# HiKapok/X-Detector

Hardware: AMD Instinct MI355X
Metric: images/sec at 480x480 Light-Head R-CNN, 1/2/4/8 MI355X + backbone MFMA util% (higher is better)
Workload: dtype f16x3 (split-precision f16 MFMA, f32 accumulate, f32 activations); 1 GPU; Full Light-Head R-CNN (Xception backbone + RPN + GPU proposals/NMS + PSROIAlign + light head + per-class NMS), 300 proposals, 480x480; batch_per_gpu=256, global_batch=256, image_size=480, concurrent_sub_batches=2, cross_terms=f16, input=whitened f32 [B,3,480,480] resident in HBM, parallelism=image-sharded dp1, weights=seeded random init (no checkpoint exists), graph_replay=True

## Files before the change

### x-detector_amd/csrc/conv_mfma_dma.hip

```cpp
#include "common.h"
#include "conv_epilogue.h"
#include <cstdlib>
#include <cstring>
#include <type_traits>

namespace xdet {

typedef float f32x16 __attribute__((ext_vector_type(16)));
typedef _Float16 f16x8 __attribute__((ext_vector_type(8)));
typedef int x8frag __attribute__((ext_vector_type(8)));
typedef int x8half __attribute__((ext_vector_type(4)));
typedef unsigned short u16;

#define XDET_GLDS16(gptr, lptr)                                                                        \
  __builtin_amdgcn_global_load_lds((const __attribute__((address_space(1))) void*)(gptr),              \
                                   (__attribute__((address_space(3))) void*)(lptr), 16, 0, 0)

template <int BM, int BN, int WAVES_M, int WAVES_N, int NSPLIT, int NSTAGE, bool PW = false, bool FOLD = false, bool X8 = false,
          bool GBUF = false>
__global__ __launch_bounds__(64 * WAVES_M * WAVES_N) void conv_dma_f16_kernel(ConvParams p_in) {
  static_assert(NSTAGE == 2, "two LDS stages");
  static_assert(!(GBUF && PW), "GBUF is the buffer form of the NON-pointwise layers");
  static_assert(!X8 || (PW && NSPLIT == 3 && !FOLD), "x8: pointwise f16x3 layers only");
  constexpr int NW = WAVES_M * WAVES_N;
  constexpr int WM = BM / WAVES_M, WN = BN / WAVES_N;
  constexpr int TM = WM / 32, TN = WN / 32;
  constexpr int A_IT = BM / (16 * NW);
  constexpr int B_IT = BN / (16 * NW);
  static_assert(A_IT >= 1 && B_IT >= 1, "tile too small for the wave count");
  constexpr int ROWB = 32;
  constexpr int STAGE = (2 * BM + 2 * BN) * ROWB;

  extern __shared__ __attribute__((aligned(16))) u16 smem16[];

  const int tid = threadIdx.x;
  const int lane = tid & 63;
  const int wave = __builtin_amdgcn_readfirstlane(tid >> 6);
  const int wm = wave / WAVES_N, wn = wave % WAVES_N;
  const int nby = p_in.Cout_pad / BN;
  const int slot = blockIdx.x >> 3;
  int bx, n0;
  ConvParams p = p_in;
  if (p_in.group_rows) {
    const int mt = p_in.group_rows / BM;
    const int tpg = mt * nby;
    const int g = (slot / tpg) * 8 + (blockIdx.x & 7);
    const int w = slot - (slot / tpg) * tpg;
    if ((int64_t)g * p_in.group_rows >= p_in.M) return;
    if (p_in.group_live_rows && (w / nby) * BM >= p_in.group_live_rows) return;
    bx = g * mt + w / nby;
    n0 = (w % nby) * BN;
    p.wt_hi = p_in.wt_hi + (size_t)g * p_in.group_wt_stride;
    p.wt_lo = p_in.wt_lo ? p_in.wt_lo + (size_t)g * p_in.group_wt_stride : nullptr;
    p.scale = p_in.scale + (size_t)g * p_in.Cout_pad;
    p.shift = p_in.shift + (size_t)g * p_in.Cout_pad;
  } else {
    bx = (slot / nby) * 8 + (blockIdx.x & 7);
    if (bx * BM >= p_in.M) return;
    n0 = (slot % nby) * BN;
  }
  const int m0 = bx * BM;

  const int lr = lane >> 2;
  const int pos = lane & 3;
  int iy0[A_IT], ix0[A_IT], pbase[A_IT], achunk[A_IT];
#pragma unroll
  for (int q = 0; q < A_IT; ++q) {
    const int rt = (wave * A_IT + q) * 16 + lr;
    achunk[q] = (pos ^ ((rt >> 2) & 3)) * 8;
    const int m = m0 + rt;
    if (m < p.M) {
      const int hw = p.Ho * p.Wo;
      const int n = m / hw;
      const int rem = m - n * hw;
      const int oy = rem / p.Wo;
      const int ox = rem - oy * p.Wo;
      iy0[q] = oy * p.stride - p.pad_t;
      ix0[q] = ox * p.stride - p.pad_l;
      pbase[q] = n * p.H * p.W;
    } else {
      iy0[q] = -(1 << 20);
      ix0[q] = 0;
      pbase[q] = 0;
    }
  }
  size_t boff[B_IT];
#pragma unroll
  for (int q = 0; q < B_IT; ++q) {
    const int rt = (wave * B_IT + q) * 16 + lr;
    boff[q] = (size_t)(n0 + rt) * 32 + (pos ^ ((rt >> 2) & 3)) * 8;
  }
  const int nk = p.Kp / 32;
  const int ntaps = p.KH * p.KW;
  const unsigned c32n = (unsigned)(p.ldi >> 5);

  __amdgpu_buffer_rsrc_t r_ah, r_al, r_bh, r_bl;
  unsigned a_vo[A_IT], b_vo[B_IT];
  int g_cc = 0, g_ky = 0, g_kx = 0, g_tap = 0;
  if (GBUF) {
    const unsigned a_bytes = (unsigned)(((size_t)(((size_t)p.N * p.H * p.W + 15) >> 4) * c32n) << 10);
    const unsigned b_bytes = (unsigned)((size_t)nk * p.Cout_pad * 64);
    r_ah = __builtin_amdgcn_make_buffer_rsrc(const_cast<u16*>(p.in_hi), 0, (int)a_bytes, 0x00020000);
    r_al = __builtin_amdgcn_make_buffer_rsrc(const_cast<u16*>(NSPLIT > 1 ? p.in_lo : p.in_hi), 0, (int)a_bytes, 0x00020000);
    r_bh = __builtin_amdgcn_make_buffer_rsrc(const_cast<u16*>(p.wt_hi), 0, (int)b_bytes, 0x00020000);
    r_bl = __builtin_amdgcn_make_buffer_rsrc(const_cast<u16*>(NSPLIT > 1 ? p.wt_lo : p.wt_hi), 0, (int)b_bytes, 0x00020000);
#pragma unroll
    for (int q = 0; q < B_IT; ++q) b_vo[q] = (unsigned)(boff[q] * 2);
  }
  if (PW) {
    const unsigned a_bytes = (unsigned)(((size_t)((p.M + 15) >> 4) * c32n) << 10);
    const unsigned b_bytes = (unsigned)((size_t)nk * p.Cout_pad * 64);
    r_ah = __builtin_amdgcn_make_buffer_rsrc(const_cast<u16*>(p.in_hi), 0, (int)a_bytes, 0x00020000);
    r_al = __builtin_amdgcn_make_buffer_rsrc(const_cast<u16*>(NSPLIT > 1 ? p.in_lo : p.in_hi), 0, (int)a_bytes, 0x00020000);
    r_bh = __builtin_amdgcn_make_buffer_rsrc(const_cast<u16*>(p.wt_hi), 0, (int)b_bytes, 0x00020000);
    r_bl = __builtin_amdgcn_make_buffer_rsrc(const_cast<u16*>(NSPLIT > 1 ? p.wt_lo : p.wt_hi), 0, (int)b_bytes, 0x00020000);
#pragma unroll
    for (int q = 0; q < A_IT; ++q) {
      const int rt = (wave * A_IT + q) * 16 + lr;
      const int m = m0 + rt;
      a_vo[q] = m < p.M ? (((unsigned)(m >> 4) * c32n) << 10) + (unsigned)((((m & 15) << 5) + achunk[q]) * 2) : 0xffffffffu;
    }
#pragma unroll
    for (int q = 0; q < B_IT; ++q) b_vo[q] = (unsigned)(boff[q] * 2);
  }

  auto issue = [&](int kt, int buf) {
    u16* Ah = smem16 + buf * STAGE;
    u16* Al = Ah + BM * ROWB;
    u16* Bh = Al + BM * ROWB;
    u16* Bl = Bh + BN * ROWB;
    if (PW) {
      const unsigned a_so = (unsigned)kt << 10;
      const unsigned b_so = (unsigned)kt * (unsigned)p.Cout_pad * 64u;
#pragma unroll
      for (int q = 0; q < A_IT; ++q) {
        __builtin_amdgcn_raw_ptr_buffer_load_lds(r_ah, (__attribute__((address_space(3))) void*)(Ah + (wave * A_IT + q) * 16 * ROWB),
                                                 16, (int)a_vo[q], (int)a_so, 0, 0);
        if (NSPLIT > 1)
          __builtin_amdgcn_raw_ptr_buffer_load_lds(r_al, (__attribute__((address_space(3))) void*)(Al + (wave * A_IT + q) * 16 * ROWB),
                                                   16, (int)a_vo[q], (int)a_so, 0, 0);
      }
#pragma unroll
      for (int q = 0; q < B_IT; ++q) {
        __builtin_amdgcn_raw_ptr_buffer_load_lds(r_bh, (__attribute__((address_space(3))) void*)(Bh + (wave * B_IT + q) * 16 * ROWB),
                                                 16, (int)b_vo[q], (int)b_so, 0, 0);
        if (NSPLIT > 1)
          __builtin_amdgcn_raw_ptr_buffer_load_lds(r_bl, (__attribute__((address_space(3))) void*)(Bl + (wave * B_IT + q) * 16 * ROWB),
                                                   16, (int)b_vo[q], (int)b_so, 0, 0);
      }
    } else if (GBUF) {
      const int dy = g_ky * p.dil, dx = g_kx * p.dil;
      const unsigned a_so = (unsigned)g_cc << 10;
      const unsigned b_so = (unsigned)(g_tap * (p.Cin_p >> 5) + g_cc) * (unsigned)p.Cout_pad * 64u;
#pragma unroll
      for (int q = 0; q < A_IT; ++q) {
        const int iy = iy0[q] + dy, ix = ix0[q] + dx;
        const bool ok = (unsigned)iy < (unsigned)p.H && (unsigned)ix < (unsigned)p.W;
        const unsigned pix = (unsigned)(pbase[q] + iy * p.W + ix);
        const unsigned vo = ok ? (((pix >> 4) * c32n) << 10) + (((pix & 15) << 5) + (unsigned)achunk[q]) * 2u : 0xffffffffu;
        __builtin_amdgcn_raw_ptr_buffer_load_lds(r_ah, (__attribute__((address_space(3))) void*)(Ah + (wave * A_IT + q) * 16 * ROWB),
                                                 16, (int)vo, (int)a_so, 0, 0);
        if (NSPLIT > 1)
          __builtin_amdgcn_raw_ptr_buffer_load_lds(r_al, (__attribute__((address_space(3))) void*)(Al + (wave * A_IT + q) * 16 * ROWB),
                                                   16, (int)vo, (int)a_so, 0, 0);
      }
#pragma unroll
      for (int q = 0; q < B_IT; ++q) {
        __builtin_amdgcn_raw_ptr_buffer_load_lds(r_bh, (__attribute__((address_space(3))) void*)(Bh + (wave * B_IT + q) * 16 * ROWB),
                                                 16, (int)b_vo[q], (int)b_so, 0, 0);
        if (NSPLIT > 1)
          __builtin_amdgcn_raw_ptr_buffer_load_lds(r_bl, (__attribute__((address_space(3))) void*)(Bl + (wave * B_IT + q) * 16 * ROWB),
                                                   16, (int)b_vo[q], (int)b_so, 0, 0);
      }
      ++g_tap;
      if (++g_kx == p.KW) {
        g_kx = 0;
        if (++g_ky == p.KH) { g_ky = 0; g_tap = 0; ++g_cc; }
      }
    } else {
    const int cc = kt / ntaps;
    const int tap = kt - cc * ntaps;
    const int ky = tap / p.KW;
    const int dy = ky * p.dil, dx = (tap - ky * p.KW) * p.dil;
    const size_t k0 = (size_t)(tap * (p.Cin_p >> 5) + cc) * p.Cout_pad * 32;
#pragma unroll
    for (int q = 0; q < A_IT; ++q) {
      const int iy = iy0[q] + dy, ix = ix0[q] + dx;
      const bool ok = (unsigned)iy < (unsigned)p.H && (unsigned)ix < (unsigned)p.W;
      const unsigned pix = (unsigned)(pbase[q] + iy * p.W + ix);
      const size_t off = ((size_t)((pix >> 4) * c32n + cc) << 9) + ((pix & 15) << 5) + achunk[q];
      const u16* sh = ok ? p.in_hi + off : p.zeros;
      XDET_GLDS16(sh, Ah + (wave * A_IT + q) * 16 * ROWB);
      if (NSPLIT > 1) {
        const u16* sl = ok ? p.in_lo + off : p.zeros;
        XDET_GLDS16(sl, Al + (wave * A_IT + q) * 16 * ROWB);
      }
    }
#pragma unroll
    for (int q = 0; q < B_IT; ++q) {
      XDET_GLDS16(p.wt_hi + boff[q] + k0, Bh + (wave * B_IT + q) * 16 * ROWB);
      if (NSPLIT > 1) XDET_GLDS16(p.wt_lo + boff[q] + k0, Bl + (wave * B_IT + q) * 16 * ROWB);
    }
    }
  };

  f32x16 acc[TM][TN];
#pragma unroll
  for (int i = 0; i < TM; ++i)
#pragma unroll
    for (int j = 0; j < TN; ++j)
#pragma unroll
      for (int r = 0; r < 16; ++r) acc[i][j][r] = 0.f;

  const int frow = lane & 31;
  const int fh = lane >> 5;
  int aoff[TM], boffs[TN], asw[TM], bsw[TN];
#pragma unroll
  for (int i = 0; i < TM; ++i) {
    const int rt = wm * WM + i * 32 + frow;
    aoff[i] = rt * ROWB;
    asw[i] = (rt >> 2) & 3;
  }
#pragma unroll
  for (int j = 0; j < TN; ++j) {
    const int rt = wn * WN + j * 32 + frow;
    boffs[j] = rt * ROWB;
    bsw[j] = (rt >> 2) & 3;
  }

  f32x16 tot[FOLD ? TM : 1][FOLD ? TN : 1];
  int fold_steps = 1 << 30, next_fold = 1 << 30;
  bool first_range = true;
  if constexpr (FOLD) {
    const int ncc = p.Cin_p >> 5, S = p.ksplit > 0 ? p.ksplit : 1;
    fold_steps = ((ncc + S - 1) / S) * ntaps;
    next_fold = fold_steps;
#pragma unroll
    for (int i = 0; i < TM; ++i)
#pragma unroll
      for (int j = 0; j < TN; ++j)
#pragma unroll
        for (int r = 0; r < 16; ++r) tot[i][j][r] = 0.f;
  }
  auto main_loop = [&](auto JN_) {
  constexpr int JN = decltype(JN_)::value;
  auto load_frags = [&](int buf, int ks, f16x8* ah, f16x8* al, f16x8* bh, f16x8* bl) {
    const u16* Ah = smem16 + buf * STAGE;
    const u16* Al = Ah + BM * ROWB;
    const u16* Bh = Al + BM * ROWB;
    const u16* Bl = Bh + BN * ROWB;
    const int c = ks * 2 + fh;
#pragma unroll
    for (int i = 0; i < TM; ++i) {
      const int o = aoff[i] + ((c ^ asw[i]) << 3);
      ah[i] = *reinterpret_cast<const f16x8*>(Ah + o);
      if constexpr (NSPLIT > 1 && !X8) al[i] = *reinterpret_cast<const f16x8*>(Al + o);
    }
#pragma unroll
    for (int j = 0; j < JN; ++j) {
      const int o = boffs[j] + ((c ^ bsw[j]) << 3);
      bh[j] = *reinterpret_cast<const f16x8*>(Bh + o);
      if constexpr (NSPLIT > 1 && !X8) bl[j] = *reinterpret_cast<const f16x8*>(Bl + o);
    }
  };
  auto load_x8 = [&](int buf, x8frag* a8, x8frag* b8) {
    const u16* Al = smem16 + buf * STAGE + BM * ROWB;
    const u16* Bl = Al + BM * ROWB + BN * ROWB;
#pragma unroll
    for (int i = 0; i < TM; ++i) {
      const x8half q0 = *reinterpret_cast<const x8half*>(Al + aoff[i] + (((2 * fh) ^ asw[i]) << 3));
      const x8half q1 = *reinterpret_cast<const x8half*>(Al + aoff[i] + (((2 * fh + 1) ^ asw[i]) << 3));
      a8[i] = x8frag{q0[0], q0[1], q0[2], q0[3], q1[0], q1[1], q1[2], q1[3]};
    }
#pragma unroll
    for (int j = 0; j < JN; ++j) {
      const x8half q0 = *reinterpret_cast<const x8half*>(Bl + boffs[j] + (((2 * fh) ^ bsw[j]) << 3));
      const x8half q1 = *reinterpret_cast<const x8half*>(Bl + boffs[j] + (((2 * fh + 1) ^ bsw[j]) << 3));
      b8[j] = x8frag{q0[0], q0[1], q0[2], q0[3], q1[0], q1[1], q1[2], q1[3]};
    }
  };
  const int x8_sa = X8 ? 127 + p.x8_exp - (fh ? 11 : 0) : 0;
  const int x8_sb = fh ? 127 + 2 : 127 - 9;
  auto mma_x8 = [&](const x8frag* a8, const x8frag* b8) {
#pragma unroll
    for (int i = 0; i < TM; ++i)
#pragma unroll
      for (int j = 0; j < JN; ++j)
        acc[i][j] = __builtin_amdgcn_mfma_scale_f32_32x32x64_f8f6f4(a8[i], b8[j], acc[i][j], 0, 0, 0, x8_sa, 0, x8_sb);
  };
  auto mma = [&](const f16x8* ah, const f16x8* al, const f16x8* bh, const f16x8* bl) {
    if constexpr (NSPLIT > 1 && !X8) {
#pragma unroll
      for (int i = 0; i < TM; ++i)
#pragma unroll
        for (int j = 0; j < JN; ++j)
          acc[i][j] = __builtin_amdgcn_mfma_f32_32x32x16_f16(al[i], bh[j], acc[i][j], 0, 0, 0);
#pragma unroll
      for (int i = 0; i < TM; ++i)
#pragma unroll
        for (int j = 0; j < JN; ++j)
          acc[i][j] = __builtin_amdgcn_mfma_f32_32x32x16_f16(ah[i], bl[j], acc[i][j], 0, 0, 0);
    }
#pragma unroll
    for (int i = 0; i < TM; ++i)
#pragma unroll
      for (int j = 0; j < JN; ++j)
        acc[i][j] = __builtin_amdgcn_mfma_f32_32x32x16_f16(ah[i], bh[j], acc[i][j], 0, 0, 0);
  };

  f16x8 a0h[TM], a0l[X8 ? 1 : TM], b0h[TN], b0l[X8 ? 1 : TN];
  f16x8 a1h[TM], a1l[X8 ? 1 : TM], b1h[TN], b1l[X8 ? 1 : TN];
  x8frag a8[X8 ? TM : 1], b8[X8 ? TN : 1];
  issue(0, 0);
  asm volatile("s_waitcnt vmcnt(0)" ::: "memory");
  __syncthreads();
  if (nk > 1) issue(1, 1);
  load_frags(0, 0, a0h, a0l, b0h, b0l);
  auto step = [&](int kt, auto steady) {
    constexpr bool STEADY = decltype(steady)::value;
    const int buf = kt & 1;
    if constexpr (FOLD) {
      if (kt == next_fold) {
#pragma unroll
        for (int i = 0; i < TM; ++i)
#pragma unroll
          for (int j = 0; j < TN; ++j) {
            tot[i][j] = first_range ? acc[i][j] : tot[i][j] + acc[i][j];
#pragma unroll
            for (int r = 0; r < 16; ++r) acc[i][j][r] = 0.f;
          }
        first_range = false;
        next_fold += fold_steps;
      }
    }
    load_frags(buf, 1, a1h, a1l, b1h, b1l);
    if constexpr (X8) load_x8(buf, a8, b8);
    __builtin_amdgcn_sched_barrier(0);
    mma(a0h, a0l, b0h, b0l);
    __builtin_amdgcn_sched_barrier(0);
    asm volatile("s_waitcnt vmcnt(0)" ::: "memory");
    __syncthreads();
    if (STEADY || kt + 1 < nk) load_frags(buf ^ 1, 0, a0h, a0l, b0h, b0l);
    if (STEADY || kt + 2 < nk) issue(kt + 2, buf);
    if (!STEADY) __builtin_amdgcn_sched_barrier(0);
    mma(a1h, a1l, b1h, b1l);
    if constexpr (X8) mma_x8(a8, b8);
    if (STEADY) {
      constexpr int NPIECE = (A_IT + B_IT) * (NSPLIT > 1 ? 2 : 1);
      constexpr int NMMA = TM * JN * (X8 ? 2 : NSPLIT > 1 ? 3 : 1);
      constexpr int NRD = (TM + JN) * (NSPLIT > 1 && !X8 ? 2 : 1);
      __builtin_amdgcn_sched_group_barrier(0x100, NRD, 0);
#pragma unroll
      for (int k = 0; k < NPIECE; ++k) {
        __builtin_amdgcn_sched_group_barrier(0x008, NMMA / NPIECE > 0 ? NMMA / NPIECE : 1, 0);
        __builtin_amdgcn_sched_group_barrier(0x010, 1, 0);
      }
    }
    __builtin_amdgcn_sched_barrier(0);
  };
  int kt = 0;
  for (; kt + 2 < nk; ++kt) step(kt, std::true_type{});
  for (; kt < nk; ++kt) step(kt, std::false_type{});
  };
  const int jn_live = (p.ldo - (n0 + wn * WN) + 31) >> 5;
  static_assert(TN == 2, "the tiles of this kernel are two column blocks per wave");
  if constexpr (PW) {
    if (jn_live == 1 && p.skip_dead != 0) main_loop(std::integral_constant<int, 1>{});
    else main_loop(std::integral_constant<int, TN>{});
  } else {
    main_loop(std::integral_constant<int, TN>{});
  }

  if constexpr (FOLD) {
    if (!first_range) {
#pragma unroll
      for (int i = 0; i < TM; ++i)
#pragma unroll
        for (int j = 0; j < TN; ++j) acc[i][j] = tot[i][j] + acc[i][j];
    }
  }
  if (m0 + BM <= p.M) conv_epilogue_full<WM, WN, TM, TN, NW, NSTAGE * STAGE * 2>(p, acc, smem16, wave, lane, wm, wn, m0, n0);
  else conv_epilogue<WM, WN, TM, TN, NW, NSTAGE * STAGE * 2>(p, acc, smem16, wave, lane, wm, wn, m0, n0);
}

template <int OFF>
__device__ __forceinline__ f16x8 cd_ds_read_b128(unsigned addr) {
  f16x8 r;
  asm volatile("ds_read_b128 %0, %1 offset:%2" : "=v"(r) : "v"(addr), "n"(OFF) : "memory");
  return r;
}

template <int NSPLIT, bool PW = false, bool W8 = false, bool H64 = false>
__global__ __launch_bounds__(W8 ? 512 : 256) void conv_dma_deep_kernel(ConvParams p_in) {
  constexpr int BM = H64 ? 64 : 128, BN = 64, NW = W8 ? 8 : 4;
  static_assert(!W8 || NSPLIT == 3, "eight waves: the f16x3 form");
  static_assert(!(W8 && H64), "64 x 64 tiles: four waves");
  constexpr bool WT = W8 || H64;
  constexpr int PAIR = 2;
  constexpr int NSTAGE = 3 * PAIR;
  constexpr int TN = WT ? 1 : 2;
  constexpr int A_IT = BM / (16 * NW), B_IT = W8 ? 1 : BN / (16 * NW);
  constexpr int ROWB = 32;
  constexpr int STAGE = (2 * BM + 2 * BN) * ROWB;
  constexpr int PIECES = W8 ? 3 : (A_IT + B_IT) * (NSPLIT > 1 ? 2 : 1);
  extern __shared__ __attribute__((aligned(16))) u16 smem16[];

  const int tid = threadIdx.x;
  const int lane = tid & 63;
  const int wave = __builtin_amdgcn_readfirstlane(tid >> 6);
  const int nby = p_in.Cout_pad / BN;
  const int slot = blockIdx.x >> 3;
  int bx, n0;
  ConvParams p = p_in;
  if (p_in.group_rows) {
    const int mt = p_in.group_rows / BM;
    const int tpg = mt * nby;
    const int g = (slot / tpg) * 8 + (blockIdx.x & 7);
    const int w = slot - (slot / tpg) * tpg;
    if ((int64_t)g * p_in.group_rows >= p_in.M) return;
    if (p_in.group_live_rows && (w / nby) * BM >= p_in.group_live_rows) return;
    bx = g * mt + w / nby;
    n0 = (w % nby) * BN;
    p.wt_hi = p_in.wt_hi + (size_t)g * p_in.group_wt_stride;
    p.wt_lo = p_in.wt_lo ? p_in.wt_lo + (size_t)g * p_in.group_wt_stride : nullptr;
    p.scale = p_in.scale + (size_t)g * p_in.Cout_pad;
    p.shift = p_in.shift + (size_t)g * p_in.Cout_pad;
  } else {
    bx = (slot / nby) * 8 + (blockIdx.x & 7);
    if (bx * BM >= p_in.M) return;
    n0 = (slot % nby) * BN;
  }
  const int m0 = bx * BM;

  const int lr = lane >> 2, pos = lane & 3;
  int iy0[A_IT], ix0[A_IT], pbase[A_IT], achunk[A_IT];
#pragma unroll
  for (int q = 0; q < A_IT; ++q) {
    const int rt = (wave * A_IT + q) * 16 + lr;
    achunk[q] = (pos ^ ((rt >> 2) & 3)) * 8;
    const int m = m0 + rt;
    if (m < p.M) {
      const int hw = p.Ho * p.Wo;
      const int n = m / hw;
      const int rem = m - n * hw;
      const int oy = rem / p.Wo;
      const int ox = rem - oy * p.Wo;
      iy0[q] = oy * p.stride - p.pad_t;
      ix0[q] = ox * p.stride - p.pad_l;
      pbase[q] = n * p.H * p.W;
    } else {
      iy0[q] = -(1 << 20);
      ix0[q] = 0;
      pbase[q] = 0;
    }
  }
  size_t boff[B_IT];
#pragma unroll
  for (int q = 0; q < B_IT; ++q) {
    const int rt = (W8 ? (wave >> 1) : wave * B_IT + q) * 16 + lr;
    boff[q] = (size_t)(n0 + rt) * 32 + (pos ^ ((rt >> 2) & 3)) * 8;
  }
  const int nk = p.Kp / 32;
  const int ntaps = p.KH * p.KW;
  const unsigned c32n = (unsigned)(p.ldi >> 5);

  unsigned a_vo[A_IT], b_vo[B_IT];
  unsigned a_bytes = 0, b_bytes = 0;
  if (PW) {
    a_bytes = (unsigned)(((size_t)((p.M + 15) >> 4) * c32n) << 10);
    b_bytes = (unsigned)((size_t)nk * p.Cout_pad * 64);
#pragma unroll
    for (int q = 0; q < A_IT; ++q) {
      const int rt = (wave * A_IT + q) * 16 + lr;
      const int m = m0 + rt;
      a_vo[q] = m < p.M ? (((unsigned)(m >> 4) * c32n) << 10) + (unsigned)((((m & 15) << 5) + achunk[q]) * 2) : 0xffffffffu;
    }
#pragma unroll
    for (int q = 0; q < B_IT; ++q) b_vo[q] = (unsigned)(boff[q] * 2);
  }

  auto issue = [&](int kt, int buf) {
    u16* Ah = smem16 + buf * STAGE;
    u16* Al = Ah + BM * ROWB;
    u16* Bh = Al + BM * ROWB;
    u16* Bl = Bh + BN * ROWB;
    const bool live = kt < nk;
    if (PW) {
      const __amdgpu_buffer_rsrc_t r_ah = __builtin_amdgcn_make_buffer_rsrc(const_cast<u16*>(p.in_hi), 0, live ? (int)a_bytes : 0, 0x00020000);
      const __amdgpu_buffer_rsrc_t r_al = __builtin_amdgcn_make_buffer_rsrc(const_cast<u16*>(NSPLIT > 1 ? p.in_lo : p.in_hi), 0, live ? (int)a_bytes : 0, 0x00020000);
      const __amdgpu_buffer_rsrc_t r_bh = __builtin_amdgcn_make_buffer_rsrc(const_cast<u16*>(p.wt_hi), 0, live ? (int)b_bytes : 0, 0x00020000);
      const __amdgpu_buffer_rsrc_t r_bl = __builtin_amdgcn_make_buffer_rsrc(const_cast<u16*>(NSPLIT > 1 ? p.wt_lo : p.wt_hi), 0, live ? (int)b_bytes : 0, 0x00020000);
      const unsigned a_so = (unsigned)kt << 10, b_so = (unsigned)kt * (unsigned)p.Cout_pad * 64u;
#pragma unroll
      for (int q = 0; q < A_IT; ++q) {
        __builtin_amdgcn_raw_ptr_buffer_load_lds(r_ah, (__attribute__((address_space(3))) void*)(Ah + (wave * A_IT + q) * 16 * ROWB), 16, (int)a_vo[q], (int)a_so, 0, 0);
        if (NSPLIT > 1)
          __builtin_amdgcn_raw_ptr_buffer_load_lds(r_al, (__attribute__((address_space(3))) void*)(Al + (wave * A_IT + q) * 16 * ROWB), 16, (int)a_vo[q], (int)a_so, 0, 0);
      }
      if constexpr (W8) {
        __builtin_amdgcn_raw_ptr_buffer_load_lds((wave & 1) ? r_bl : r_bh, (__attribute__((address_space(3))) void*)(((wave & 1) ? Bl : Bh) + (wave >> 1) * 16 * ROWB), 16,
                                                 (int)b_vo[0], (int)b_so, 0, 0);
      } else {
#pragma unroll
      for (int q = 0; q < B_IT; ++q) {
        __builtin_amdgcn_raw_ptr_buffer_load_lds(r_bh, (__attribute__((address_space(3))) void*)(Bh + (wave * B_IT + q) * 16 * ROWB), 16, (int)b_vo[q], (int)b_so, 0, 0);
        if (NSPLIT > 1)
          __builtin_amdgcn_raw_ptr_buffer_load_lds(r_bl, (__attribute__((address_space(3))) void*)(Bl + (wave * B_IT + q) * 16 * ROWB), 16, (int)b_vo[q], (int)b_so, 0, 0);
      }
      }
    } else {
    const int cc = kt / ntaps;
    const int tap = kt - cc * ntaps;
    const int ky = tap / p.KW;
    const int dy = ky * p.dil, dx = (tap - ky * p.KW) * p.dil;
    const size_t k0 = (size_t)(tap * (p.Cin_p >> 5) + cc) * p.Cout_pad * 32;
#pragma unroll
    for (int q = 0; q < A_IT; ++q) {
      const int iy = iy0[q] + dy, ix = ix0[q] + dx;
      const bool ok = live && (unsigned)iy < (unsigned)p.H && (unsigned)ix < (unsigned)p.W;
      const unsigned pix = (unsigned)(pbase[q] + iy * p.W + ix);
      const size_t off = ((size_t)((pix >> 4) * c32n + cc) << 9) + ((pix & 15) << 5) + achunk[q];
      XDET_GLDS16(ok ? p.in_hi + off : p.zeros, Ah + (wave * A_IT + q) * 16 * ROWB);
      if (NSPLIT > 1) XDET_GLDS16(ok ? p.in_lo + off : p.zeros, Al + (wave * A_IT + q) * 16 * ROWB);
    }
    if constexpr (W8) {
      XDET_GLDS16(live ? ((wave & 1) ? p.wt_lo : p.wt_hi) + boff[0] + k0 : p.zeros, ((wave & 1) ? Bl : Bh) + (wave >> 1) * 16 * ROWB);
    } else {
#pragma unroll
    for (int q = 0; q < B_IT; ++q) {
      XDET_GLDS16(live ? p.wt_hi + boff[q] + k0 : p.zeros, Bh + (wave * B_IT + q) * 16 * ROWB);
      if (NSPLIT > 1) XDET_GLDS16(live ? p.wt_lo + boff[q] + k0 : p.zeros, Bl + (wave * B_IT + q) * 16 * ROWB);
    }
    }
    }
  };

  f32x16 acc[1][TN];
#pragma unroll
  for (int j = 0; j < TN; ++j)
#pragma unroll
    for (int r = 0; r < 16; ++r) acc[0][j][r] = 0.f;

  const int frow = lane & 31, fh = lane >> 5;
  const unsigned lds0 = (unsigned)(size_t)(__attribute__((address_space(3))) void*)(smem16);
  unsigned a_off[2], b_off[2][TN];
#pragma unroll
  for (int ks = 0; ks < 2; ++ks) {
    const int c = ks * 2 + fh;
    const int ra = (WT ? (wave >> 1) : wave) * 32 + frow;
    a_off[ks] = (unsigned)(ra * ROWB + ((c ^ ((ra >> 2) & 3)) << 3)) * 2u;
#pragma unroll
    for (int j = 0; j < TN; ++j) {
      const int rb = (WT ? (wave & 1) : j) * 32 + frow;
      b_off[ks][j] = (unsigned)(2 * BM * ROWB + rb * ROWB + ((c ^ ((rb >> 2) & 3)) << 3)) * 2u;
    }
  }

#pragma unroll
  for (int q = 0; q < 2 * PAIR; ++q) issue(q, q);
  int ring = 0;
  for (int kt = 0; kt < nk; kt += PAIR) {
    asm volatile("s_waitcnt vmcnt(%0)\n\ts_barrier" ::"n"(PAIR * PIECES) : "memory");
    {
      const int ns = ring + 2 * PAIR >= NSTAGE ? ring + 2 * PAIR - NSTAGE : ring + 2 * PAIR;
#pragma unroll
      for (int q = 0; q < PAIR; ++q) issue(kt + 2 * PAIR + q, ns + q);
    }
    __builtin_amdgcn_sched_barrier(0);
#pragma unroll
    for (int q = 0; q < PAIR; ++q) {
      const unsigned sb = lds0 + (unsigned)((ring + q) * STAGE * 2);
      f16x8 ah[2], al[2], bh[2][TN], bl[2][TN];
#pragma unroll
      for (int ks = 0; ks < 2; ++ks) {
        ah[ks] = cd_ds_read_b128<0>(sb + a_off[ks]);
        if (NSPLIT > 1) al[ks] = cd_ds_read_b128<BM * ROWB * 2>(sb + a_off[ks]);
#pragma unroll
        for (int j = 0; j < TN; ++j) {
          bh[ks][j] = cd_ds_read_b128<0>(sb + b_off[ks][j]);
          if (NSPLIT > 1) bl[ks][j] = cd_ds_read_b128<BN * ROWB * 2>(sb + b_off[ks][j]);
        }
      }
#pragma unroll
      for (int ks = 0; ks < 2; ++ks) {
        if (NSPLIT > 1) asm volatile("s_waitcnt lgkmcnt(0)" : "+v"(ah[ks]), "+v"(al[ks])::"memory");
        else asm volatile("s_waitcnt lgkmcnt(0)" : "+v"(ah[ks])::"memory");
#pragma unroll
        for (int j = 0; j < TN; ++j) {
          asm volatile("" : "+v"(bh[ks][j]));
          if (NSPLIT > 1) asm volatile("" : "+v"(bl[ks][j]));
        }
      }
#pragma unroll
      for (int ks = 0; ks < 2; ++ks) {
        if (NSPLIT > 1) {
#pragma unroll
          for (int j = 0; j < TN; ++j) acc[0][j] = __builtin_amdgcn_mfma_f32_32x32x16_f16(al[ks], bh[ks][j], acc[0][j], 0, 0, 0);
#pragma unroll
          for (int j = 0; j < TN; ++j) acc[0][j] = __builtin_amdgcn_mfma_f32_32x32x16_f16(ah[ks], bl[ks][j], acc[0][j], 0, 0, 0);
        }
#pragma unroll
        for (int j = 0; j < TN; ++j) acc[0][j] = __builtin_amdgcn_mfma_f32_32x32x16_f16(ah[ks], bh[ks][j], acc[0][j], 0, 0, 0);
      }
    }
    ring = ring + PAIR >= NSTAGE ? ring + PAIR - NSTAGE : ring + PAIR;
  }
  asm volatile("s_waitcnt vmcnt(0)" ::: "memory");
  if (m0 + BM <= p.M) conv_epilogue_full<32, 32 * TN, 1, TN, NW, NSTAGE * STAGE * 2>(p, acc, smem16, wave, lane, WT ? (wave >> 1) : wave, WT ? (wave & 1) : 0, m0, n0);
  else conv_epilogue<32, 32 * TN, 1, TN, NW, NSTAGE * STAGE * 2>(p, acc, smem16, wave, lane, WT ? (wave >> 1) : wave, WT ? (wave & 1) : 0, m0, n0);
}

static bool pw_eligible(const ConvParams& p) {
  if (p.KH != 1 || p.KW != 1 || p.stride != 1 || p.pad_t != 0 || p.pad_l != 0 || p.H != p.Ho || p.W != p.Wo) return false;
  const size_t a_bytes = ((size_t)((p.M + 15) >> 4) * (size_t)(p.ldi >> 5)) << 10;
  const size_t b_bytes = (size_t)(p.Kp / 32) * p.Cout_pad * 64;
  return a_bytes < ((size_t)1 << 32) && b_bytes < ((size_t)1 << 32) && p.Cin_p == p.Kp;
}

template <int NSPLIT, bool PW = false, bool W8 = false, bool H64 = false>
static int launch_deep(const ConvParams& p, hipStream_t s) {
  if (!PW && pw_eligible(p)) return launch_deep<NSPLIT, true, W8, H64>(p, s);
  if constexpr (!W8 && !H64 && NSPLIT == 3) {
    if (!p.group_rows && cdiv(p.M, 128) * (p.Cout_pad / 64) <= 128) return launch_deep<NSPLIT, PW, false, true>(p, s);
    return launch_deep<NSPLIT, PW, true>(p, s);
  }
  constexpr int BM = H64 ? 64 : 128;
  constexpr size_t lds = (size_t)6 * (2 * BM + 2 * 64) * 32 * sizeof(u16);
  auto kern = conv_dma_deep_kernel<NSPLIT, PW, W8, H64>;
  static DeviceOnce once;
  XDET_TRY(ensure_dynamic_lds(once, reinterpret_cast<const void*>(kern), (int)lds));
  dim3 grid((unsigned)(cdiv(cdiv(p.M, BM), 8) * 8 * (p.Cout_pad / 64)));
  if (p.group_rows) {
    const int64_t groups = p.M / p.group_rows, tpg = (int64_t)(p.group_rows / BM) * (p.Cout_pad / 64);
    grid = dim3((unsigned)(cdiv(groups, 8) * 8 * tpg));
  }
  hipLaunchKernelGGL(kern, grid, dim3(W8 ? 512 : 256), lds, s, p);
  XDET_LAUNCH_CHECK();
  return XDET_OK;
}

static bool gbuf_eligible(const ConvParams& p) {
  if (p.group_rows != 0) return false;
  const size_t a_bytes = ((((size_t)p.N * p.H * p.W + 15) >> 4) * (size_t)(p.ldi >> 5)) << 10;
  const size_t b_bytes = (size_t)(p.Kp / 32) * p.Cout_pad * 64;
  return a_bytes < ((size_t)1 << 32) && b_bytes < ((size_t)1 << 32) && p.Kp == p.Cin_p * p.KH * p.KW;
}

template <int BM, int BN, int WAVES_M, int WAVES_N, int NSPLIT, int NSTAGE = 2, bool PW = false, bool X8 = false, bool GBUF = false>
static int launch_d(const ConvParams& p, hipStream_t s) {
  if (!PW && pw_eligible(p)) return launch_d<BM, BN, WAVES_M, WAVES_N, NSPLIT, NSTAGE, true>(p, s);
  if constexpr (PW && !X8 && NSPLIT == 3) {
    if (p.x8) return launch_d<BM, BN, WAVES_M, WAVES_N, NSPLIT, NSTAGE, true, true>(p, s);
  }
  XDET_REQUIRE(X8 || !p.x8, "conv(dma): x8 planes need a pointwise f16x3 layer below 4 GiB");
  constexpr size_t lds = (size_t)NSTAGE * (2 * BM + 2 * BN) * 32 * sizeof(u16);
  if constexpr (!PW && !X8 && !GBUF && BM == 256 && BN == 256) {
    if (gbuf_eligible(p)) return launch_d<BM, BN, WAVES_M, WAVES_N, NSPLIT, NSTAGE, false, false, true>(p, s);
  }
  auto kern = conv_dma_f16_kernel<BM, BN, WAVES_M, WAVES_N, NSPLIT, NSTAGE, PW, false, X8, GBUF>;
  static DeviceOnce once;
  XDET_TRY(ensure_dynamic_lds(once, reinterpret_cast<const void*>(kern), (int)lds));
  dim3 grid((unsigned)(cdiv(cdiv(p.M, BM), 8) * 8 * (p.Cout_pad / BN)));
  if (p.group_rows) {
    const int64_t groups = p.M / p.group_rows, tpg = (int64_t)(p.group_rows / BM) * (p.Cout_pad / BN);
    grid = dim3((unsigned)(cdiv(groups, 8) * 8 * tpg));
  }
  hipLaunchKernelGGL(kern, grid, dim3(64 * WAVES_M * WAVES_N), lds, s, p);
  XDET_LAUNCH_CHECK();
  return XDET_OK;
}

bool conv_dma_fold_applicable(const ConvParams& p, int n_tile, int nsplit) {
  return n_tile == 128 && nsplit == 3 && p.group_rows == 0 && p.ksplit > 1 && cdiv(p.M, 256) * (p.Cout_pad / 128) >= 170;
}
int launch_conv_mfma_dma_fold(const ConvParams& p, hipStream_t s) {
  constexpr size_t lds = (size_t)2 * (2 * 256 + 2 * 128) * 32 * sizeof(u16);
  auto kern = conv_dma_f16_kernel<256, 128, 4, 2, 3, 2, false, true>;
  static DeviceOnce once;
  XDET_TRY(ensure_dynamic_lds(once, reinterpret_cast<const void*>(kern), (int)lds));
  dim3 grid((unsigned)(cdiv(cdiv(p.M, 256), 8) * 8 * (p.Cout_pad / 128)));
  hipLaunchKernelGGL(kern, grid, dim3(512), lds, s, p);
  XDET_LAUNCH_CHECK();
  return XDET_OK;
}

int launch_conv_mfma_dma(const ConvParams& p_in, int n_tile, int nsplit, hipStream_t s) {
  ConvParams p = p_in;
  p.skip_dead = 1;
  XDET_REQUIRE(p.Kp % 32 == 0 && p.Cin_p % 32 == 0 && p.ldi >= p.Cin_p && p.ldi % 8 == 0,
               "conv(dma): channel counts must be padded to 32");
  XDET_REQUIRE(p.Cout_pad % n_tile == 0, "conv(dma): Cout_pad must be a multiple of the N tile");
  XDET_REQUIRE(p.in_hi && (nsplit == 1 || p.in_lo) && p.wt_hi && (nsplit == 1 || p.wt_lo) && p.zeros,
               "conv(dma): split planes missing");
  if (p.M <= 0) return XDET_OK;
  if (n_tile == 128 && nsplit == 3) {
    const int64_t b256 = cdiv(p.M, 256) * (p.Cout_pad / 256);
    const int nk = p.Kp / 32;
    int tile = 0;
    const bool full_rounds = b256 >= 240 && (b256 % 256 == 0 || b256 % 256 >= 240);
    if (p.Cout_pad % 256 == 0 && (b256 >= 512 || full_rounds || (b256 >= 200 && nk >= 40))) tile = 2;
    if (p.group_rows && p.group_rows % 256 != 0) tile = 0;
    if (tile == 2) return launch_d<256, 256, 2, 4, 3>(p, s);
  }
  if (n_tile == 128 && nsplit == 3 && !p.group_rows && !p.x8) {
    const int64_t b128 = cdiv(p.M, 128) * (p.Cout_pad / 128);
    if (b128 > 128 && b128 <= 256 && p.Kp / 32 >= 16 && p.Kp == p.Cin_p * p.KH * p.KW && p.ldi % 32 == 0 &&
        conv_ksplit_supported(p.KH, p.KW, (int64_t)p.N * p.H * p.W, p.ldi, p.Cin_p, p.Cout_pad)) {
      ConvParams q = p;
      q.ksplit = 1;
      q.ks_partial = nullptr;
      return launch_conv_mfma_ksplit(q, 128, 3, 2, 0, s);
    }
  }
  if (n_tile == 128 && nsplit == 3 && p.group_rows && p.group_rows % 64 == 0 && !p.x8) {
    const int live = p.group_live_rows ? p.group_live_rows : p.group_rows;
    const int64_t groups = p.M / p.group_rows, wgs = groups * cdiv(live, 64) * (p.Cout_pad / 64);
    if (live <= 64 && wgs <= 768) return launch_deep<3, false, false, true>(p, s);
  }
  if (n_tile == 128) {
    const int64_t b128 = cdiv(p.M, 128) * (p.Cout_pad / 128);
    if (nsplit == 3 && b128 <= 128 && (!p.group_rows || p.group_rows % 128 == 0)) {
      return p.x8 ? launch_d<128, 64, 4, 1, 3>(p, s) : launch_deep<3>(p, s);
    }
    return nsplit == 1 ? launch_d<128, 128, 2, 2, 1>(p, s) : launch_d<128, 128, 2, 2, 3>(p, s);
  }
  if (n_tile == 64) return nsplit == 1 ? launch_d<128, 64, 4, 1, 1>(p, s) : launch_d<128, 64, 4, 1, 3>(p, s);
  set_last_error("conv(dma): unsupported N tile");
  return XDET_ERR_UNSUPPORTED;
}

}
```

Measured before the change: 3986 images/sec.

## Make 256x256 buffer-form conv kernels persistent, prefetching the next tile during the epilogue

For the 256x256 pointwise and buffer-form conv kernels, the launch now uses a persistent grid sized to the CU count. Each workgroup walks a strided sequence of tiles and issues the next tile's first k-slab loads before running the current tile's epilogue, with the epilogue staging moved to a separate LDS region. This targets per-workgroup launch and ramp cost and the idle memory pipe during epilogues, at the price of more LDS per workgroup (which can reduce occupancy) and extra scalar work reloading epilogue params from kernarg. It also adds optional timing-probe instrumentation behind a compile-time flag.

Result: faster. 4043 images/sec, median of 6 (+1.4%).

```diff
diff --git a/x-detector_amd/csrc/conv_mfma_dma.hip b/x-detector_amd/csrc/conv_mfma_dma.hip
--- a/x-detector_amd/csrc/conv_mfma_dma.hip
+++ b/x-detector_amd/csrc/conv_mfma_dma.hip
@@ -6,6 +6,11 @@
 
 namespace xdet {
 
+#if CD_PROBE_LEVEL == 1
+unsigned long long* g_conv_dma_probe = nullptr;
+int g_conv_dma_probe_no_walk = 0;
+#endif
+
 typedef float f32x16 __attribute__((ext_vector_type(16)));
 typedef _Float16 f16x8 __attribute__((ext_vector_type(8)));
 typedef int x8frag __attribute__((ext_vector_type(8)));
@@ -16,12 +21,44 @@
   __builtin_amdgcn_global_load_lds((const __attribute__((address_space(1))) void*)(gptr),              \
                                    (__attribute__((address_space(3))) void*)(lptr), 16, 0, 0)
 
+#ifndef CD_PROBE_LEVEL
+#define CD_PROBE_LEVEL 0
+#endif
+#if CD_PROBE_LEVEL == 1
+#define CD_PROBE_PARAM , unsigned long long* dbg
+#define CD_PROBE_ARG , g_conv_dma_probe
+#define CD_STAMP(vblk, slot)                                                      \
+  do {                                                                            \
+    if (dbg && threadIdx.x == 0) {                                                \
+      dbg[((size_t)(vblk) * 5 + (slot)) * 2] = __builtin_amdgcn_s_memrealtime();  \
+      dbg[((size_t)(vblk) * 5 + (slot)) * 2 + 1] = __builtin_amdgcn_s_memtime();  \
+    }                                                                             \
+  } while (0)
+#define CD_STAMP_DRAINED(vblk, slot)                        \
+  do {                                                      \
+    asm volatile("s_waitcnt vmcnt(0)" ::: "memory");        \
+    CD_STAMP(vblk, slot);                                   \
+  } while (0)
+#else
+#define CD_PROBE_PARAM
+#define CD_PROBE_ARG
+#define CD_STAMP(vblk, slot) do {} while (0)
+#define CD_STAMP_DRAINED(vblk, slot) do {} while (0)
+#endif
+
+constexpr int conv_dma_lds_bytes(int bm, int bn, int waves_m, int waves_n, bool walk) {
+  const int stage = (2 * bm + 2 * bn) * 32 * 2;
+  const int staging = waves_m * waves_n * 32 * (bn / waves_n + 4) * 4;
+  return walk && stage + staging > 2 * stage ? stage + staging : 2 * stage;
+}
+
 template <int BM, int BN, int WAVES_M, int WAVES_N, int NSPLIT, int NSTAGE, bool PW = false, bool FOLD = false, bool X8 = false,
-          bool GBUF = false>
-__global__ __launch_bounds__(64 * WAVES_M * WAVES_N) void conv_dma_f16_kernel(ConvParams p_in) {
+          bool GBUF = false, bool WALK = false>
+__global__ __launch_bounds__(64 * WAVES_M * WAVES_N) void conv_dma_f16_kernel(ConvParams p_in, int nvb CD_PROBE_PARAM) {
   static_assert(NSTAGE == 2, "two LDS stages");
   static_assert(!(GBUF && PW), "GBUF is the buffer form of the NON-pointwise layers");
   static_assert(!X8 || (PW && NSPLIT == 3 && !FOLD), "x8: pointwise f16x3 layers only");
+  static_assert(!WALK || ((PW || GBUF) && !FOLD), "the tile walk: the buffer forms (their weights are aimed per tile through a resource)");
   constexpr int NW = WAVES_M * WAVES_N;
   constexpr int WM = BM / WAVES_M, WN = BN / WAVES_N;
   constexpr int TM = WM / 32, TN = WN / 32;
@@ -30,6 +67,9 @@
   static_assert(A_IT >= 1 && B_IT >= 1, "tile too small for the wave count");
   constexpr int ROWB = 32;
   constexpr int STAGE = (2 * BM + 2 * BN) * ROWB;
+  constexpr int EP_OFF = WALK ? STAGE : 0;
+  constexpr int EP_BYTES = conv_dma_lds_bytes(BM, BN, WAVES_M, WAVES_N, WALK) - EP_OFF * 2;
+  static_assert(conv_dma_lds_bytes(BM, BN, WAVES_M, WAVES_N, WALK) <= 160 * 1024, "stages + epilogue staging must fit a CU's LDS");
 
   extern __shared__ __attribute__((aligned(16))) u16 smem16[];
 
@@ -38,58 +78,46 @@
   const int wave = __builtin_amdgcn_readfirstlane(tid >> 6);
   const int wm = wave / WAVES_N, wn = wave % WAVES_N;
   const int nby = p_in.Cout_pad / BN;
-  const int slot = blockIdx.x >> 3;
-  int bx, n0;
   ConvParams p = p_in;
-  if (p_in.group_rows) {
-    const int mt = p_in.group_rows / BM;
-    const int tpg = mt * nby;
-    const int g = (slot / tpg) * 8 + (blockIdx.x & 7);
-    const int w = slot - (slot / tpg) * tpg;
-    if ((int64_t)g * p_in.group_rows >= p_in.M) return;
-    if (p_in.group_live_rows && (w / nby) * BM >= p_in.group_live_rows) return;
-    bx = g * mt + w / nby;
-    n0 = (w % nby) * BN;
-    p.wt_hi = p_in.wt_hi + (size_t)g * p_in.group_wt_stride;
-    p.wt_lo = p_in.wt_lo ? p_in.wt_lo + (size_t)g * p_in.group_wt_stride : nullptr;
-    p.scale = p_in.scale + (size_t)g * p_in.Cout_pad;
-    p.shift = p_in.shift + (size_t)g * p_in.Cout_pad;
+  auto tile_of = [&](int vb, int& tm0, int& tn0, int& tg) -> bool {
+    const int slot = vb >> 3;
+    if (p_in.group_rows) {
+      const int mt = p_in.group_rows / BM;
+      const int tpg = mt * nby;
+      const int g = (slot / tpg) * 8 + (vb & 7);
+      const int w = slot - (slot / tpg) * tpg;
+      if ((int64_t)g * p_in.group_rows >= p_in.M) return false;
+      if (p_in.group_live_rows && (w / nby) * BM >= p_in.group_live_rows) return false;
+      tm0 = (g * mt + w / nby) * BM;
+      tn0 = (w % nby) * BN;
+      tg = g;
+    } else {
+      const int bx = (slot / nby) * 8 + (vb & 7);
+      if (bx * BM >= p_in.M) return false;
+      tm0 = bx * BM;
+      tn0 = (slot % nby) * BN;
+      tg = 0;
+    }
+    return true;
+  };
+  int vb = blockIdx.x;
+  int m0, n0, grp;
+  if constexpr (WALK) {
+    while (vb < nvb && !tile_of(vb, m0, n0, grp)) vb += gridDim.x;
+    if (vb >= nvb) return;
   } else {
-    bx = (slot / nby) * 8 + (blockIdx.x & 7);
-    if (bx * BM >= p_in.M) return;
-    n0 = (slot % nby) * BN;
-  }
-  const int m0 = bx * BM;
-
-  const int lr = lane >> 2;
-  const int pos = lane & 3;
+    if (!tile_of(vb, m0, n0, grp)) return;
+  }
+  if (!WALK && p_in.group_rows) {
+    p.wt_hi = p_in.wt_hi + (size_t)grp * p_in.group_wt_stride;
+    p.wt_lo = p_in.wt_lo ? p_in.wt_lo + (size_t)grp * p_in.group_wt_stride : nullptr;
+    p.scale = p_in.scale + (size_t)grp * p_in.Cout_pad;
+    p.shift = p_in.shift + (size_t)grp * p_in.Cout_pad;
+  }
+  CD_STAMP(vb, 0);
+
   int iy0[A_IT], ix0[A_IT], pbase[A_IT], achunk[A_IT];
-#pragma unroll
-  for (int q = 0; q < A_IT; ++q) {
-    const int rt = (wave * A_IT + q) * 16 + lr;
-    achunk[q] = (pos ^ ((rt >> 2) & 3)) * 8;
-    const int m = m0 + rt;
-    if (m < p.M) {
-      const int hw = p.Ho * p.Wo;
-      const int n = m / hw;
-      const int rem = m - n * hw;
-      const int oy = rem / p.Wo;
-      const int ox = rem - oy * p.Wo;
-      iy0[q] = oy * p.stride - p.pad_t;
-      ix0[q] = ox * p.stride - p.pad_l;
-      pbase[q] = n * p.H * p.W;
-    } else {
-      iy0[q] = -(1 << 20);
-      ix0[q] = 0;
-      pbase[q] = 0;
-    }
-  }
   size_t boff[B_IT];
-#pragma unroll
-  for (int q = 0; q < B_IT; ++q) {
-    const int rt = (wave * B_IT + q) * 16 + lr;
-    boff[q] = (size_t)(n0 + rt) * 32 + (pos ^ ((rt >> 2) & 3)) * 8;
-  }
   const int nk = p.Kp / 32;
   const int ntaps = p.KH * p.KW;
   const unsigned c32n = (unsigned)(p.ldi >> 5);
@@ -97,32 +125,55 @@
   __amdgpu_buffer_rsrc_t r_ah, r_al, r_bh, r_bl;
   unsigned a_vo[A_IT], b_vo[B_IT];
   int g_cc = 0, g_ky = 0, g_kx = 0, g_tap = 0;
-  if (GBUF) {
-    const unsigned a_bytes = (unsigned)(((size_t)(((size_t)p.N * p.H * p.W + 15) >> 4) * c32n) << 10);
-    const unsigned b_bytes = (unsigned)((size_t)nk * p.Cout_pad * 64);
+  if (PW || GBUF) {
+    const unsigned a_bytes = GBUF ? (unsigned)(((size_t)(((size_t)p.N * p.H * p.W + 15) >> 4) * c32n) << 10)
+                                  : (unsigned)(((size_t)((p.M + 15) >> 4) * c32n) << 10);
     r_ah = __builtin_amdgcn_make_buffer_rsrc(const_cast<u16*>(p.in_hi), 0, (int)a_bytes, 0x00020000);
     r_al = __builtin_amdgcn_make_buffer_rsrc(const_cast<u16*>(NSPLIT > 1 ? p.in_lo : p.in_hi), 0, (int)a_bytes, 0x00020000);
-    r_bh = __builtin_amdgcn_make_buffer_rsrc(const_cast<u16*>(p.wt_hi), 0, (int)b_bytes, 0x00020000);
-    r_bl = __builtin_amdgcn_make_buffer_rsrc(const_cast<u16*>(NSPLIT > 1 ? p.wt_lo : p.wt_hi), 0, (int)b_bytes, 0x00020000);
-#pragma unroll
-    for (int q = 0; q < B_IT; ++q) b_vo[q] = (unsigned)(boff[q] * 2);
-  }
-  if (PW) {
-    const unsigned a_bytes = (unsigned)(((size_t)((p.M + 15) >> 4) * c32n) << 10);
-    const unsigned b_bytes = (unsigned)((size_t)nk * p.Cout_pad * 64);
-    r_ah = __builtin_amdgcn_make_buffer_rsrc(const_cast<u16*>(p.in_hi), 0, (int)a_bytes, 0x00020000);
-    r_al = __builtin_amdgcn_make_buffer_rsrc(const_cast<u16*>(NSPLIT > 1 ? p.in_lo : p.in_hi), 0, (int)a_bytes, 0x00020000);
-    r_bh = __builtin_amdgcn_make_buffer_rsrc(const_cast<u16*>(p.wt_hi), 0, (int)b_bytes, 0x00020000);
-    r_bl = __builtin_amdgcn_make_buffer_rsrc(const_cast<u16*>(NSPLIT > 1 ? p.wt_lo : p.wt_hi), 0, (int)b_bytes, 0x00020000);
+  }
+  auto aim = [&](int ln, int tm0, int tn0, int tg) {
+    const int lr = ln >> 2;
+    const int pos = ln & 3;
 #pragma unroll
     for (int q = 0; q < A_IT; ++q) {
       const int rt = (wave * A_IT + q) * 16 + lr;
-      const int m = m0 + rt;
-      a_vo[q] = m < p.M ? (((unsigned)(m >> 4) * c32n) << 10) + (unsigned)((((m & 15) << 5) + achunk[q]) * 2) : 0xffffffffu;
-    }
-#pragma unroll
-    for (int q = 0; q < B_IT; ++q) b_vo[q] = (unsigned)(boff[q] * 2);
-  }
+      achunk[q] = (pos ^ ((rt >> 2) & 3)) * 8;
+      const int m = tm0 + rt;
+      if (!PW) {
+        if (m < p.M) {
+          int hw = p.Ho * p.Wo, wo = p.Wo;
+          if (WALK) asm volatile("" : "+s"(hw), "+s"(wo));
+          const int n = m / hw;
+          const int rem = m - n * hw;
+          const int oy = rem / wo;
+          const int ox = rem - oy * wo;
+          iy0[q] = oy * p.stride - p.pad_t;
+          ix0[q] = ox * p.stride - p.pad_l;
+          pbase[q] = n * p.H * p.W;
+        } else {
+          iy0[q] = -(1 << 20);
+          ix0[q] = 0;
+          pbase[q] = 0;
+        }
+      } else {
+        a_vo[q] = m < p.M ? (((unsigned)(m >> 4) * c32n) << 10) + (unsigned)((((m & 15) << 5) + achunk[q]) * 2) : 0xffffffffu;
+      }
+    }
+#pragma unroll
+    for (int q = 0; q < B_IT; ++q) {
+      const int rt = (wave * B_IT + q) * 16 + lr;
+      boff[q] = (size_t)(tn0 + rt) * 32 + (pos ^ ((rt >> 2) & 3)) * 8;
+      if (PW || GBUF) b_vo[q] = (unsigned)(boff[q] * 2);
+    }
+    if (PW || GBUF) {
+      const size_t wo = WALK ? (size_t)tg * p_in.group_wt_stride : 0;
+      const unsigned b_bytes = (unsigned)((size_t)nk * p.Cout_pad * 64);
+      r_bh = __builtin_amdgcn_make_buffer_rsrc(const_cast<u16*>(p.wt_hi + wo), 0, (int)b_bytes, 0x00020000);
+      r_bl = __builtin_amdgcn_make_buffer_rsrc(const_cast<u16*>((NSPLIT > 1 ? p.wt_lo : p.wt_hi) + wo), 0, (int)b_bytes, 0x00020000);
+    }
+    g_cc = g_ky = g_kx = g_tap = 0;
+  };
+  aim(lane, m0, n0, grp);
 
   auto issue = [&](int kt, int buf) {
     u16* Ah = smem16 + buf * STAGE;
@@ -205,15 +256,27 @@
   };
 
   f32x16 acc[TM][TN];
-#pragma unroll
-  for (int i = 0; i < TM; ++i)
-#pragma unroll
-    for (int j = 0; j < TN; ++j)
-#pragma unroll
-      for (int r = 0; r < 16; ++r) acc[i][j][r] = 0.f;
-
-  const int frow = lane & 31;
-  const int fh = lane >> 5;
+  bool more = false;
+  int m0_nx = 0, n0_nx = 0, grp_nx = 0;
+  int lane_t = lane;
+  auto next_tile = [&]() {
+    vb += gridDim.x;
+    while (vb < nvb && !tile_of(vb, m0_nx, n0_nx, grp_nx)) vb += gridDim.x;
+    if (vb < nvb) {
+      more = true;
+      aim(lane_t, m0_nx, n0_nx, grp_nx);
+      issue(0, 0);
+    }
+  };
+  int vbc = vb;
+  (void)vbc;
+  bool first_tile = true;
+  issue(0, 0);
+  do {
+  more = false;
+  if (WALK) lane_t = ep_lane();
+  const int frow = lane_t & 31;
+  const int fh = lane_t >> 5;
   int aoff[TM], boffs[TN], asw[TM], bsw[TN];
 #pragma unroll
   for (int i = 0; i < TM; ++i) {
@@ -227,6 +290,14 @@
     boffs[j] = rt * ROWB;
     bsw[j] = (rt >> 2) & 3;
   }
+
+  if (WALK && PW) aim(lane_t, m0, n0, grp);
+#pragma unroll
+  for (int i = 0; i < TM; ++i)
+#pragma unroll
+    for (int j = 0; j < TN; ++j)
+#pragma unroll
+      for (int r = 0; r < 16; ++r) acc[i][j][r] = 0.f;
 
   f32x16 tot[FOLD ? TM : 1][FOLD ? TN : 1];
   int fold_steps = 1 << 30, next_fold = 1 << 30;
@@ -311,9 +382,9 @@
   f16x8 a0h[TM], a0l[X8 ? 1 : TM], b0h[TN], b0l[X8 ? 1 : TN];
   f16x8 a1h[TM], a1l[X8 ? 1 : TM], b1h[TN], b1l[X8 ? 1 : TN];
   x8frag a8[X8 ? TM : 1], b8[X8 ? TN : 1];
-  issue(0, 0);
-  asm volatile("s_waitcnt vmcnt(0)" ::: "memory");
+  if (!WALK || first_tile) asm volatile("s_waitcnt vmcnt(0)" ::: "memory");
   __syncthreads();
+  CD_STAMP(vbc, 1);
   if (nk > 1) issue(1, 1);
   load_frags(0, 0, a0h, a0l, b0h, b0l);
   auto step = [&](int kt, auto steady) {
@@ -342,6 +413,7 @@
     __syncthreads();
     if (STEADY || kt + 1 < nk) load_frags(buf ^ 1, 0, a0h, a0l, b0h, b0l);
     if (STEADY || kt + 2 < nk) issue(kt + 2, buf);
+    else if (WALK && kt + 1 == nk) next_tile();
     if (!STEADY) __builtin_amdgcn_sched_barrier(0);
     mma(a1h, a1l, b1h, b1l);
     if constexpr (X8) mma_x8(a8, b8);
@@ -379,8 +451,33 @@
         for (int j = 0; j < TN; ++j) acc[i][j] = tot[i][j] + acc[i][j];
     }
   }
-  if (m0 + BM <= p.M) conv_epilogue_full<WM, WN, TM, TN, NW, NSTAGE * STAGE * 2>(p, acc, smem16, wave, lane, wm, wn, m0, n0);
-  else conv_epilogue<WM, WN, TM, TN, NW, NSTAGE * STAGE * 2>(p, acc, smem16, wave, lane, wm, wn, m0, n0);
+  CD_STAMP(vbc, 2);
+  if constexpr (WALK) {
+    const __attribute__((address_space(4))) ConvParams* kp =
+        (const __attribute__((address_space(4))) ConvParams*)__builtin_amdgcn_kernarg_segment_ptr();
+    asm volatile("" : "+s"(kp));
+    ConvParams pe = {};
+    pe.out = kp->out; pe.out_hi = kp->out_hi; pe.out_lo = kp->out_lo; pe.res = kp->res;
+    pe.planes_relu = kp->planes_relu; pe.pl_c32 = kp->pl_c32; pe.pl_scale = kp->pl_scale; pe.pl_shift = kp->pl_shift;
+    pe.ldo = kp->ldo; pe.ldr = kp->ldr; pe.M = kp->M; pe.relu_out = kp->relu_out;
+    pe.scale = kp->scale + (size_t)grp * kp->Cout_pad;
+    pe.shift = kp->shift + (size_t)grp * kp->Cout_pad;
+    asm volatile("s_waitcnt vmcnt(0)" ::: "memory");
+    if (m0 + BM <= pe.M) conv_epilogue_full<WM, WN, TM, TN, NW, EP_BYTES>(pe, acc, smem16 + EP_OFF, wave, lane, wm, wn, m0, n0);
+    else conv_epilogue<WM, WN, TM, TN, NW, EP_BYTES>(pe, acc, smem16 + EP_OFF, wave, lane, wm, wn, m0, n0);
+  } else {
+    if (m0 + BM <= p.M) conv_epilogue_full<WM, WN, TM, TN, NW, EP_BYTES>(p, acc, smem16 + EP_OFF, wave, lane, wm, wn, m0, n0);
+    else conv_epilogue<WM, WN, TM, TN, NW, EP_BYTES>(p, acc, smem16 + EP_OFF, wave, lane, wm, wn, m0, n0);
+  }
+  CD_STAMP(vbc, 3);
+  CD_STAMP_DRAINED(vbc, 4);
+  m0 = m0_nx;
+  n0 = n0_nx;
+  grp = grp_nx;
+  vbc = vb;
+  first_tile = false;
+  if (more) CD_STAMP(vbc, 0);
+  } while (WALK && more);
 }
 
 template <int OFF>
@@ -646,6 +743,19 @@
   return a_bytes < ((size_t)1 << 32) && b_bytes < ((size_t)1 << 32) && p.Kp == p.Cin_p * p.KH * p.KW;
 }
 
+static int device_cu_count(int* n_out) {
+  static std::atomic<int> cus[64];
+  int dev = 0;
+  XDET_HIP(hipGetDevice(&dev));
+  int n = cus[dev & 63].load(std::memory_order_acquire);
+  if (n <= 0) {
+    XDET_HIP(hipDeviceGetAttribute(&n, hipDeviceAttributeMultiprocessorCount, dev));
+    cus[dev & 63].store(n, std::memory_order_release);
+  }
+  *n_out = n;
+  return XDET_OK;
+}
+
 template <int BM, int BN, int WAVES_M, int WAVES_N, int NSPLIT, int NSTAGE = 2, bool PW = false, bool X8 = false, bool GBUF = false>
 static int launch_d(const ConvParams& p, hipStream_t s) {
   if (!PW && pw_eligible(p)) return launch_d<BM, BN, WAVES_M, WAVES_N, NSPLIT, NSTAGE, true>(p, s);
@@ -653,19 +763,37 @@
     if (p.x8) return launch_d<BM, BN, WAVES_M, WAVES_N, NSPLIT, NSTAGE, true, true>(p, s);
   }
   XDET_REQUIRE(X8 || !p.x8, "conv(dma): x8 planes need a pointwise f16x3 layer below 4 GiB");
-  constexpr size_t lds = (size_t)NSTAGE * (2 * BM + 2 * BN) * 32 * sizeof(u16);
+  constexpr size_t lds = conv_dma_lds_bytes(BM, BN, WAVES_M, WAVES_N, false);
   if constexpr (!PW && !X8 && !GBUF && BM == 256 && BN == 256) {
     if (gbuf_eligible(p)) return launch_d<BM, BN, WAVES_M, WAVES_N, NSPLIT, NSTAGE, false, false, true>(p, s);
+  }
+  int64_t nvb = cdiv(cdiv(p.M, BM), 8) * 8 * (p.Cout_pad / BN);
+  if (p.group_rows) {
+    const int64_t groups = p.M / p.group_rows, tpg = (int64_t)(p.group_rows / BM) * (p.Cout_pad / BN);
+    nvb = cdiv(groups, 8) * 8 * tpg;
+  }
+  if constexpr (BM == 256 && BN == 256 && (PW || GBUF)) {
+    int cus = 0;
+    XDET_TRY(device_cu_count(&cus));
+    const int64_t wgs = cus / 8 * 8;
+    bool walk = wgs >= 8 && nvb > wgs;
+#if CD_PROBE_LEVEL == 1
+    if (g_conv_dma_probe_no_walk) walk = false;
+#endif
+    if (walk) {
+      constexpr size_t lds_w = conv_dma_lds_bytes(BM, BN, WAVES_M, WAVES_N, true);
+      auto kern_w = conv_dma_f16_kernel<BM, BN, WAVES_M, WAVES_N, NSPLIT, NSTAGE, PW, false, X8, GBUF, true>;
+      static DeviceOnce once_w;
+      XDET_TRY(ensure_dynamic_lds(once_w, reinterpret_cast<const void*>(kern_w), (int)lds_w));
+      hipLaunchKernelGGL(kern_w, dim3((unsigned)wgs), dim3(64 * WAVES_M * WAVES_N), lds_w, s, p, (int)nvb CD_PROBE_ARG);
+      XDET_LAUNCH_CHECK();
+      return XDET_OK;
+    }
   }
   auto kern = conv_dma_f16_kernel<BM, BN, WAVES_M, WAVES_N, NSPLIT, NSTAGE, PW, false, X8, GBUF>;
   static DeviceOnce once;
   XDET_TRY(ensure_dynamic_lds(once, reinterpret_cast<const void*>(kern), (int)lds));
-  dim3 grid((unsigned)(cdiv(cdiv(p.M, BM), 8) * 8 * (p.Cout_pad / BN)));
-  if (p.group_rows) {
-    const int64_t groups = p.M / p.group_rows, tpg = (int64_t)(p.group_rows / BM) * (p.Cout_pad / BN);
-    grid = dim3((unsigned)(cdiv(groups, 8) * 8 * tpg));
-  }
-  hipLaunchKernelGGL(kern, grid, dim3(64 * WAVES_M * WAVES_N), lds, s, p);
+  hipLaunchKernelGGL(kern, dim3((unsigned)nvb), dim3(64 * WAVES_M * WAVES_N), lds, s, p, (int)nvb CD_PROBE_ARG);
   XDET_LAUNCH_CHECK();
   return XDET_OK;
 }
@@ -679,7 +807,7 @@
   static DeviceOnce once;
   XDET_TRY(ensure_dynamic_lds(once, reinterpret_cast<const void*>(kern), (int)lds));
   dim3 grid((unsigned)(cdiv(cdiv(p.M, 256), 8) * 8 * (p.Cout_pad / 128)));
-  hipLaunchKernelGGL(kern, grid, dim3(512), lds, s, p);
+  hipLaunchKernelGGL(kern, grid, dim3(512), lds, s, p, (int)grid.x CD_PROBE_ARG);
   XDET_LAUNCH_CHECK();
   return XDET_OK;
 }
```
